# CederGroupHub/sparse-lm

Measured on NVIDIA B200. Metric: cv_grid_fits_per_sec, higher is better.
Workload: dtype f64

## Files before the change

### sparselm_b200/csrc/engine.cu

```cuda
#include <cuda_runtime.h>
#include <float.h>
#include <math.h>
#include <stdint.h>
#include <stdio.h>
#include <stdlib.h>
#include <string.h>

#include <algorithm>
#include <string>
#include <vector>

#include "../../include/sparselm_b200.h"
#include "gemm_f64.cuh"
#include "gemm_f64_tma.cuh"
#include "solver_kernels.cuh"
#include "whiten_kernels.cuh"
#include "cg_kernels.cuh"
#include "coop_kernels.cuh"
#include "newton_kernels.cuh"
#include "select_kernels.cuh"

using namespace slm;

enum { FAM_GRAM = 0, FAM_APPLY = 1, FAM_PROX = 2, FAM_GAP = 3, FAM_SCORE = 4, FAM_LIPS = 5, FAM_COUNT = 6 };
// ... 1776 lines not shown
            LAUNCH_OK("zflags_kernel");
        }
        const bool probe = can_adapt && !check && !coop && !clus && (it == 1 || it == 3 || it == 6);
        const int cw_now = (wide && !check && !probe) ? cw_wide : cw;
        const double* ap_in = fused ? Bc[par] : Z;
        double* ap_out = fused ? GBc[par] : GZ;
        int rc = sparse ? apply_rowsparse(ctx, sp, Kcur, ap_in, ap_out, cw_now, (int)((ldz + cw_now - 1) / cw_now), sidx,
                                          scount, s, algo)
                        : apply_batched(ctx, bt->G_dev, bt->g_stride, bt->pa, p, F, Kcur, ap_in, ldz, ap_out, s, algo);
        if (rc) return rc;
        if ((check || probe) && (can_adapt || (clus_thr > 0 && sparse && F * ncc <= kMaxScount)))
            CUDA_OK(cudaMemcpyAsync(ctx->h_scount, scount, sizeof(int) * (size_t)F * ncc, cudaMemcpyDeviceToHost, s));
        if (probe) {
            CUDA_OK(cudaStreamSynchronize(s));
            decide_width();
        }
        if (check) {
            CUDA_OK(cudaMemsetAsync(ctx->d_counter, 0, sizeof(int) * SLM_MAX_FOLDS, s));
            CUDA_OK(cudaMemsetAsync(ctx->d_ratio, 0, sizeof(unsigned long long), s));
            {
                FamTimer tm(ctx, FAM_GAP, s, 0.0);
                SolveDev spg = sp;
                if (fused) {
                    spg.B = Bc[par];
                    spg.GZ = GBc[par];
                    spg.direct = 1;
                }
                if (grouped)
                    gap_partial_kernel<true><<<cgrid, ST, 0, s>>>(spg, par, 0);
                else
                    gap_partial_kernel<false><<<cgrid, ST, 0, s>>>(spg, par, 0);
                gap_final_kernel<<<fgrid, 128, 0, s>>>(spg, it, 0);
                if (fused) settle_done_kernel<<<mgrid, ST, 0, s>>>(sp, Bc[par], Bc[par ^ 1]);
            }
            LAUNCH_OK("gap kernels");
            ctx->launches++;
            CUDA_OK(cudaMemcpyAsync(ctx->h_counter, ctx->d_counter, sizeof(int) * SLM_MAX_FOLDS,
                                    cudaMemcpyDeviceToHost, s));
            CUDA_OK(cudaMemcpyAsync(ctx->h_ratio, ctx->d_ratio, sizeof(unsigned long long),
                                    cudaMemcpyDeviceToHost, s));
            CUDA_OK(cudaStreamSynchronize(s));
            n_active = 0;
            bool shrink = false;
            for (int f = 0; f < F; ++f) {
                n_active_f[f] = ctx->h_counter[f];
                n_active += n_active_f[f];
                if (round_up(n_active_f[f], 8) < round_up(Kcur[f], 8)) shrink = true;
            }
            next_regular = it + ((n_active * 8 <= Ktot && Ktot >= 16) ? std::max(2, check_every / 2) : check_every);
            if (ctx->trace)
                fprintf(stderr, "[slm] it=%d active=%lld Kmax=%d%s\n", it, n_active, Kmax,
                        coop ? " coop" : (small ? " small" : (clus ? " cluster" : "")));
            if (n_active == 0) break;
            if (clus_thr > 0) {
                bool pays = false;
                if (n_active <= clus_thr && sparse && F * ncc <= kMaxScount) {
                    double bytes = 0.0, flops = 0.0;
                    for (int f = 0; f < F; ++f) {
                        const int Kp = (int)std::min<int64_t>(round_up(n_active_f[f], 8), ldz);
                        for (int cc = 0; cc * cw < Kp; ++cc) {
                            const double sc = (double)std::min<long long>(ctx->h_scount[f * ncc + cc], p);
                            const double ncol = (double)std::min(cw, Kp - cc * cw);
                            bytes += ncol * (double)p * sc * 8.0;
                            flops += 2.0 * ncol * (double)p * sc;
                        }
                    }
                    const int conc = std::max(1, std::min(ctx->sm_count / clus_cs_min, 8 * (16 / clus_cs_min)));
                    const double rounds = (double)((n_active + conc - 1) / conc);
                    const double t_cl = std::max(rounds * 12e-6, bytes / 3.0e12);
                    const double t_ge = 90e-6 + flops / 20e12;
                    pays = t_cl < 0.5 * t_ge;
                }
                if (pays && !clus) {
                    clus = true;
                    interval = check_every;
                    prev_ratio = 0.0;
                } else if (!pays && clus) {
                    clus = false;
                }
            }
            do_compact = shrink && !small && !coop;
            if (small || coop || clus) {
                int step_to = interval;
                double ratio;
                memcpy(&ratio, ctx->h_ratio, sizeof(double));
                if (prev_ratio > 0.0 && ratio > 1.0 && ratio < prev_ratio && it > prev_check) {
                    const double rate = log(prev_ratio / ratio) / (double)(it - prev_check);
                    const double need = 1.15 * log(ratio) / rate + 1.0;
                    if (need < (double)step_to) step_to = std::max(std::max(2, check_every / 2), (int)ceil(need));
                }
                prev_ratio = ratio;
                prev_check = it;
                next_check = it + step_to;
                interval = std::min(interval * 2, 2048);
            }
            if (can_adapt) decide_width();
        }
        {
            FamTimer tm(ctx, FAM_PROX, s, 0.0);
            if (fused) {
                FusedArgs fa;
                fa.Bcur = Bc[par];
                fa.Bnew = Bc[par ^ 1];
                fa.GBcur = GBc[par];
                fa.GBold = GBc[par ^ 1];
                fa.stash = Z;
                fa.it = it;
                fa.use_rst = use_rst;
                use_rst = 0;
                const int rows_lane = bt->max_group > 0 ? (bt->max_group + SUB - 1) / SUB : 8;
                if (!grouped)
                    prox_fused_kernel<false, 1><<<cgrid, ST, 0, s>>>(sp, fa, par);
                else if (rows_lane <= 2)
                    prox_fused_kernel<true, 2><<<cgrid, ST, 0, s>>>(sp, fa, par);
                else if (rows_lane <= 3)
                    prox_fused_kernel<true, 3><<<cgrid, ST, 0, s>>>(sp, fa, par);
                else if (rows_lane <= 5)
                    prox_fused_kernel<true, 5><<<cgrid, ST, 0, s>>>(sp, fa, par);
                else
                    prox_fused_kernel<true, 8><<<cgrid, ST, 0, s>>>(sp, fa, par);
            } else if (ctx->prox2) {
                SolveDev s2 = sp;
                s2.gpt = std::max(1, (Gn + PX_W * kMaxChunks - 1) / (PX_W * kMaxChunks));
                s2.n_chunks = (Gn + PX_W * s2.gpt - 1) / (PX_W * s2.gpt);
                const dim3 cgrid2((unsigned)((Kmax + PX_C - 1) / PX_C), (unsigned)s2.n_chunks, (unsigned)F);
                const dim3 mgrid2((unsigned)((Kmax + PX_C - 1) / PX_C), (unsigned)((p + MOM_ROWS - 1) / MOM_ROWS),
                                  (unsigned)F);
                if (grouped)
                    prox_main2_kernel<true><<<cgrid2, PX_W * PX_C, 0, s>>>(s2, par);
                else
                    prox_main2_kernel<false><<<cgrid2, PX_W * PX_C, 0, s>>>(s2, par);
                prox_momentum2_kernel<<<mgrid2, PX_W * PX_C, 0, s>>>(s2, par);
            } else {
                if (grouped)
                    prox_main_kernel<true><<<cgrid, ST, 0, s>>>(sp, par);
                else
                    prox_main_kernel<false><<<cgrid, ST, 0, s>>>(sp, par);
                prox_momentum_kernel<<<mgrid, ST, 0, s>>>(sp, par);
            }
        }
        LAUNCH_OK("prox kernels");
        ctx->launches++;
        if (do_compact) {
            SolveDev spc = sp;
            if (fused) {
                spc.Z = Bc[par ^ 1];
                spc.B = Bc[par];
                spc.GB = GBc[par];
                restart_reduce_kernel<<<fgrid, 128, 0, s>>>(sp, par);
                use_rst = 1;
            }
            compact_plan_kernel<<<F, 32, 0, s>>>(sp, src, newK);
            scatter_done_kernel<<<mgrid, ST, 0, s>>>(spc, 0);
            compact_move_kernel<<<dim3((unsigned)((p + 127) / 128), 3, (unsigned)F), 128, 0, s>>>(spc, src, newK);
            compact_cols_kernel<<<F, 32, 0, s>>>(sp, src, newK, colmap);
            LAUNCH_OK("compaction kernels");
            ctx->launches += 3;
            Kmax = 0;
            for (int f = 0; f < F; ++f) {
                sp.K[f] = Kcur[f] = n_active_f[f];
                Kmax = std::max(Kmax, Kcur[f]);
            }
            grids(Kmax, cgrid, mgrid, fgrid);
            do_compact = false;
            if (sparse) {
                zflags_kernel<<<zgrid, 256, 0, s>>>(sp, fused ? Bc[par ^ 1] : Z);
                LAUNCH_OK("zflags_kernel");
            }
        }
        if (fused && clus) {
            const int pn = par ^ 1;
            fused_to_classic_kernel<<<mgrid, ST, 0, s>>>(sp, Bc[pn], Bc[par], GBc[par], it + 1, pn, use_rst);
            LAUNCH_OK("fused_to_classic_kernel");
            use_rst = 0;
            fused = false;
            if (sparse) {
                zflags_kernel<<<zgrid, 256, 0, s>>>(sp, Z);
                LAUNCH_OK("zflags_kernel");
            }
        }
    }
    bt->iters_run = it;
    {
        SolveDev spe = sp;
        if (fused) spe.B = Bc[it & 1];
        scatter_done_kernel<<<mgrid, ST, 0, s>>>(spe, 1);
    }
    LAUNCH_OK("scatter_done_kernel");

    SolveDev fin = sp;
    fin.B = bt->B_dev;
    fin.colmap = nullptr;
    for (int f = 0; f < F; ++f) fin.K[f] = bt->K[f];
    grids(Kmax0, cgrid, mgrid, fgrid);
    CUDA_OK(cudaMemcpyAsync(Z, bt->B_dev, state * sizeof(double), cudaMemcpyDeviceToDevice, s));
    if (sparse) {
        zflags_kernel<<<zgrid, 256, 0, s>>>(fin, Z);
        LAUNCH_OK("zflags_kernel");
        int rc = apply_rowsparse(ctx, fin, bt->K, Z, GZ, cw, ncc, sidx, scount, s, 0.0);
        if (rc) return rc;
        CUDA_OK(cudaMemcpyAsync(ctx->h_stat, ctx->d_stat, sizeof(unsigned long long), cudaMemcpyDeviceToHost, s));
    } else {
        int rc = apply_batched(ctx, bt->G_dev, bt->g_stride, bt->pa, p, F, bt->K, Z, ldz, GZ, s, 0.0);
        if (rc) return rc;
    }
    CUDA_OK(cudaMemsetAsync(ctx->d_counter, 0, sizeof(int) * SLM_MAX_FOLDS, s));
    {
        FamTimer tm(ctx, FAM_GAP, s, 0.0);
        if (grouped)
            gap_partial_kernel<true><<<cgrid, ST, 0, s>>>(fin, 0, 1);
        else
            gap_partial_kernel<false><<<cgrid, ST, 0, s>>>(fin, 0, 1);
        gap_final_kernel<<<fgrid, 128, 0, s>>>(fin, it, 1);
    }
    LAUNCH_OK("gap kernels(final)");
    ctx->launches++;
    CUDA_OK(cudaMemcpyAsync(ctx->h_counter, ctx->d_counter, sizeof(int) * SLM_MAX_FOLDS, cudaMemcpyDeviceToHost, s));
    CUDA_OK(cudaStreamSynchronize(s));
    bt->n_unconverged = 0;
    for (int f = 0; f < F; ++f) bt->n_unconverged += ctx->h_counter[f];
    if (sparse) ctx->apply_exec_flops += 2.0 * (double)p * (double)(*ctx->h_stat);
    return 0;
}


static inline int64_t nw_ldh(int64_t p) { return round_up(p, 8); }
static inline int nw_panels(int64_t p) { return (int)((p + NW_NB - 1) / NW_NB); }

size_t slm_newton_workspace(int64_t p, int32_t n_groups, int32_t k, int n_folds) {
    const size_t ldh = (size_t)nw_ldh(p), kk = (size_t)k;
    const size_t ldz = (size_t)round_up(k, 8);
    size_t d = kk * ldh * ldh;
    d += kk * (size_t)nw_panels(p) * NW_NB * NW_NB;
    d += 6 * kk * ldh;
    d += (size_t)round_up((int64_t)(kk * (size_t)n_groups), 2);
    d += 2 * (size_t)n_folds * (size_t)p * ldz;
    return d * sizeof(double) + (4 * kk + kk * ldh + 64) * sizeof(int) + 256;
}

static int newton_step_impl(slm_ctx* ctx, const double* G, int64_t g_stride, int64_t pa, int64_t p, int n_folds,
                            int32_t k, const int32_t* fold_host, const double* nobs_dev, double* X, const double* W2,
                            const double* D2, const double* W1, const int32_t* gptr, const int32_t* gid,
                            int32_t n_groups, void* work, size_t work_bytes, double* out, void* stream) {
    if (!ctx || !G || !fold_host || !nobs_dev || !X || !W2 || !gptr || !gid || !work || !out)
        return fail(ctx, 1, "slm_newton_step: null argument");
    if (k <= 0) return 0;
    if (n_folds < 1 || n_folds > SLM_MAX_FOLDS) return fail(ctx, 1, "slm_newton_step: n_folds out of range");
    if (work_bytes < slm_newton_workspace(p, n_groups, k, n_folds))
        return fail(ctx, 1, "slm_newton_step: workspace too small");
    if (n_groups > 6000) return fail(ctx, 1, "slm_newton_step: too many groups for the line-search kernel");
    cudaStream_t s = (cudaStream_t)stream;
    const int64_t ldv = nw_ldh(p), ldz = round_up(k, 8);
    double* H = (double*)work;
    double* INV = H + (size_t)k * ldv * ldv;
    double* U = INV + (size_t)k * nw_panels(p) * NW_NB * NW_NB;
    double* KK = U + (size_t)k * ldv;
    double* DP = KK + (size_t)k * ldv;
    double* GS = DP + (size_t)k * ldv;
    double* GRAD = GS + (size_t)k * ldv;
    double* DIR = GRAD + (size_t)k * ldv;
    double* NRM = DIR + (size_t)k * ldv;
    double* Z = NRM + (size_t)round_up((int64_t)k * n_groups, 2);
    double* GZ = Z + (size_t)n_folds * p * ldz;
    int* fold_dev = (int*)(GZ + (size_t)n_folds * p * ldz);
    int* slot_dev = fold_dev + k;
    int* info = slot_dev + k;
    int* MS = info + k;
    int* ACT = MS + k;

    std::vector<int32_t> fs(2 * (size_t)k), Kf(n_folds, 0);
    for (int c = 0; c < k; ++c) {
        const int f = fold_host[c];
        if (f < 0 || f >= n_folds) return fail(ctx, 1, "slm_newton_step: fold index out of range");
        fs[c] = f;
        fs[k + c] = Kf[f]++;
    }
    CUDA_OK(cudaMemcpyAsync(fold_dev, fs.data(), sizeof(int32_t) * 2 * (size_t)k, cudaMemcpyHostToDevice, s));
    CUDA_OK(cudaMemsetAsync(info, 0, sizeof(int) * (size_t)k, s));
    CUDA_OK(cudaMemsetAsync(Z, 0, sizeof(double) * (size_t)n_folds * p * ldz, s));

    if (!ctx->newton_smem_set) {
        CUDA_OK(cudaFuncSetAttribute(chol_diag_kernel, cudaFuncAttributeMaxDynamicSharedMemorySize, (int)NW_TILE_SMEM));
        CUDA_OK(cudaFuncSetAttribute(chol_panel_kernel, cudaFuncAttributeMaxDynamicSharedMemorySize, (int)NW_TILE_SMEM));
        CUDA_OK(cudaFuncSetAttribute(newton_linesearch_kernel, cudaFuncAttributeMaxDynamicSharedMemorySize, 98304));
        CUDA_OK(cudaFuncSetAttribute(chol_solve_kernel, cudaFuncAttributeMaxDynamicSharedMemorySize, 98304));
        ctx->newton_smem_set = true;
    }
    const dim3 vgrid((unsigned)((p + NW_T - 1) / NW_T), (unsigned)k);
    newton_prepare_kernel<<<k, NW_T, 0, s>>>((int)p, n_groups, gptr, X, ldv, W2, D2, W1, NRM, U, KK, DP, ACT, MS);
    std::vector<int> ms((size_t)k);
    CUDA_OK(cudaMemcpyAsync(ms.data(), MS, sizeof(int) * (size_t)k, cudaMemcpyDeviceToHost, s));
    newton_pack_kernel<<<vgrid, NW_T, 0, s>>>((int)p, fold_dev, slot_dev, X, ldv, Z, ldz);
    LAUNCH_OK("newton prepare/pack kernels");
    if (int rc = apply_batched(ctx, G, g_stride, pa, p, n_folds, Kf.data(), Z, ldz, GZ, s, -1.0, FAM_LIPS)) return rc;
    newton_grad_kernel<<<vgrid, NW_T, 0, s>>>((int)p, G, g_stride, pa, fold_dev, slot_dev, nobs_dev, X, GZ, ldz, ldv, KK,
                                              DP, W1, GS, GRAD);
    CUDA_OK(cudaStreamSynchronize(s));
    int m_max = 0;
    for (int c = 0; c < k; ++c) m_max = std::max(m_max, ms[c]);
    const int64_t ldh = std::max<int64_t>(8, nw_ldh(m_max));
    const int npan = std::max(1, nw_panels(m_max));
    if (m_max > 0) {
        const dim3 hgrid((unsigned)((ldh + NW_T - 1) / NW_T), (unsigned)ldh, (unsigned)k);
        newton_hessian_kernel<<<hgrid, NW_T, 0, s>>>((int)p, G, g_stride, pa, fold_dev, nobs_dev, gid, U, KK, DP, ldv, ACT, MS,
                                                     H, ldh);
    }
    LAUNCH_OK("newton grad/hessian kernels");
// ... 378 lines not shown
```

### sparselm_b200/csrc/solver_kernels.cuh

```cuda
#pragma once
#include <cuda_runtime.h>
#include <math.h>

#include "../../include/sparselm_b200.h"

namespace slm {

#ifndef SLM_PROX_UR
#define SLM_PROX_UR 1
#endif
#ifndef SLM_PROX_MINB
#define SLM_PROX_MINB 4
#endif
constexpr int SC = 8;
constexpr int SG = 32;
constexpr int ST = SC * SG;
constexpr int kMaxChunks = 64;
constexpr int NQ = 7;
constexpr int MOM_ROWS = 256;

struct SolveDev {
    int F, p, Gn;
    int gpt;
    int n_chunks;
// ... 553 lines not shown
                const int j = j0 + r;
                if (j < jb) {
                    const long long e = sbase + (long long)j * ldz;
                    const double gb = (gz[r] + theta * gbo[r]) * inv1pt;
                    const double v = z[r] - son * (gz[r] - cj[r]);
                    const double u = softt(v, step * w1[r]);
                    if (active) {
                        sp.GB[e] = gb;
                        sp.T[e] = u;
                    }
                    ss += u * u;
                }
            }
        }
        const double nrm = sqrt(ss);
        const double w2 = sp.W2 ? sp.W2[gbase + (long long)g * ldz] : 0.0;
        const double d2 = sp.D2 ? sp.D2[gbase + (long long)g * ldz] : 0.0;
        double scale = nrm > 0.0 ? fmax(0.0, 1.0 - step * w2 / nrm) : 0.0;
        scale = scale / (1.0 + step * d2);
        if (active) {
            for (int j0 = ja; j0 < jb; j0 += PX_UR) {
                double t[PX_UR], z[PX_UR], bo[PX_UR];
#pragma unroll
                for (int r = 0; r < PX_UR; ++r) {
                    const int j = j0 + r;
                    if (j < jb) {
                        const long long e = sbase + (long long)j * ldz;
                        t[r] = sp.T[e];
                        z[r] = sp.Z[e];
                        bo[r] = sp.B[e];
                    }
                }
#pragma unroll
                for (int r = 0; r < PX_UR; ++r) {
                    const int j = j0 + r;
                    if (j < jb) {
                        const double bn = scale * t[r];
                        sp.T[sbase + (long long)j * ldz] = bn;
                        dot += (z[r] - bn) * (bn - bo[r]);
                    }
                }
            }
        }
    }
    red[w][lane] = active ? dot : 0.0;
    __syncthreads();
    if (w == 0 && active) {
        double d = 0.0;
#pragma unroll
        for (int q = 0; q < PX_W; ++q) d += red[q][lane];
        sp.part[(((long long)f * sp.n_chunks + chunk) * NQ + 0) * ldz + k] = d;
    }
}

__global__ void __launch_bounds__(PX_W * PX_C) prox_momentum2_kernel(const __grid_constant__ SolveDev sp, int par) {
    const int f = blockIdx.z;
    const int Kf = sp.K[f];
    const int k0 = blockIdx.x * PX_C;
    if (k0 >= Kf) return;
    const int lane = threadIdx.x & 31, w = threadIdx.x >> 5;
    const int k = k0 + lane;
    const long long ldz = sp.ldz;
    const long long colbase = (long long)f * ldz + k;
    const bool active = (k < Kf) && sp.flag[colbase] == 0;
    const int j0 = blockIdx.y * MOM_ROWS;
    const int j1 = min(j0 + MOM_ROWS, sp.p);
    const int cb0 = blockIdx.x * (PX_C / SC);
    if (__syncthreads_and(!active)) {
        if (sp.zflag)
            for (int e = threadIdx.x; e < (j1 - j0) * (PX_C / SC); e += PX_W * PX_C) {
                const int j = j0 + e / (PX_C / SC), cb = cb0 + e % (PX_C / SC);
                if (cb < sp.nblk) sp.zflag[((long long)f * sp.p + j) * sp.nblk + cb] = 0;
            }
        return;
    }
    double dsum = 0.0;
    if (active)
        for (int ch = 0; ch < sp.n_chunks; ++ch) dsum += sp.part[(((long long)f * sp.n_chunks + ch) * NQ + 0) * ldz + k];
    const double tm = active ? sp.tmom[par][colbase] : 1.0;
    double tn = 0.5 * (1.0 + sqrt(1.0 + 4.0 * tm * tm));
    double th = (tm - 1.0) / tn;
    if (dsum > 0.0) {
        th = 0.0;
        tn = 1.0;
    }
    const long long sbase = (long long)f * sp.p * ldz + k;
#pragma unroll 1
    for (int jj = w; jj < MOM_ROWS; jj += 4 * PX_W) {
        double bn[4], b[4];
        bool inb[4];
#pragma unroll
        for (int r = 0; r < 4; ++r) {
            const int j = j0 + jj + r * PX_W;
            inb[r] = j < j1;
            if (inb[r] && active) {
                const long long e = sbase + (long long)j * ldz;
                bn[r] = sp.T[e];
                b[r] = sp.B[e];
            }
        }
#pragma unroll
        for (int r = 0; r < 4; ++r) {
            const int j = j0 + jj + r * PX_W;
            bool nz = false;
            if (inb[r] && active) {
                const long long e = sbase + (long long)j * ldz;
                const double z = bn[r] + th * (bn[r] - b[r]);
                sp.Z[e] = z;
                sp.B[e] = bn[r];
                nz = z != 0.0;
            }
            if (sp.zflag) {
                const unsigned bal = __ballot_sync(0xffffffffu, nz);
                if ((lane & 7) == 0 && inb[r]) {
                    const int cb = cb0 + (lane >> 3);
                    if (cb < sp.nblk)
                        sp.zflag[((long long)f * sp.p + j) * sp.nblk + cb] = (unsigned char)(((bal >> lane) & 0xffu) != 0u);
                }
            }
        }
    }
    if (active && blockIdx.y == 0 && w == 0) {
        sp.theta[par ^ 1][colbase] = th;
        sp.tmom[par ^ 1][colbase] = tn;
    }
}

__global__ void __launch_bounds__(256) zflags_kernel(const __grid_constant__ SolveDev sp,
                                                     const double* __restrict__ Zsrc) {
    const int f = blockIdx.y;
    const long long i = (long long)blockIdx.x * blockDim.x + threadIdx.x;
    if (i >= (long long)sp.p * sp.nblk) return;
    const int j = (int)(i / sp.nblk), cb = (int)(i - (long long)j * sp.nblk);
    const int Kf = sp.K[f];
    bool nz = false;
    const double* row = Zsrc + ((long long)f * sp.p + j) * sp.ldz;
    for (int k = cb * SC; k < min(cb * SC + SC, Kf); ++k) nz |= row[k] != 0.0;
    sp.zflag[((long long)f * sp.p + j) * sp.nblk + cb] = nz ? 1 : 0;
}

__global__ void __launch_bounds__(1024) support_list_kernel(const __grid_constant__ SolveDev sp, int wb, int ncc,
                                                            int* __restrict__ sidx, int* __restrict__ scount,
                                                            unsigned long long* __restrict__ stat) {
    const int f = blockIdx.y, cc = blockIdx.x;
    const int Kf = sp.K[f];
    const int nb_f = (Kf + SC - 1) / SC;
    const int b0 = cc * wb, b1 = min(b0 + wb, nb_f);
    const int tid = threadIdx.x, lane = tid & 31, warp = tid >> 5;
    int* out = sidx + ((long long)f * ncc + cc) * sp.p;
    if (b0 >= nb_f) {
        if (tid == 0) scount[f * ncc + cc] = 0;
        return;
    }
    __shared__ int wtot[32];
    __shared__ int woff[32];
    __shared__ int base_s, btot;
    if (tid == 0) base_s = 0;
    __syncthreads();
    for (int j0 = 0; j0 < sp.p; j0 += 1024) {
        const int j = j0 + tid;
        bool nz = false;
        if (j < sp.p) {
            const unsigned char* fl = sp.zflag + ((long long)f * sp.p + j) * sp.nblk;
            for (int b = b0; b < b1; ++b) nz |= fl[b] != 0;
        }
        const unsigned bal = __ballot_sync(0xffffffffu, nz);
        if (lane == 0) wtot[warp] = __popc(bal);
        __syncthreads();
        if (warp == 0) {
            int v = wtot[lane], x = v;
#pragma unroll
            for (int o = 1; o < 32; o <<= 1) {
                int y = __shfl_up_sync(0xffffffffu, x, o);
                if (lane >= o) x += y;
            }
            woff[lane] = x - v;
            if (lane == 31) btot = x;
        }
        __syncthreads();
        const int base = base_s;
        if (nz) out[base + woff[warp] + __popc(bal & ((1u << lane) - 1u))] = j;
        __syncthreads();
        if (tid == 0) base_s = base + btot;
        __syncthreads();
    }
    if (tid == 0) {
        scount[f * ncc + cc] = base_s;
        if (stat) atomicAdd(stat, (unsigned long long)base_s * (unsigned long long)(min(b1 * SC, Kf) - b0 * SC));
    }
}

template <bool GROUPED, typename GF, typename WF>
__device__ __forceinline__ double group_dual_newton(unsigned qmask, int ja, int jb, int sub, int rstep, double w2,
                                                    double lo, double hi, GF gfun, WF wfun) {
    double nu = lo;
    for (int it = 0; it < 50; ++it) {
        double s2 = 0.0, sw = 0.0;
        for (int j = ja + sub; j < jb; j += rstep) {
            const double w = wfun(j);
            const double u = gfun(j) - nu * w;
            if (u > 0.0) {
                s2 += u * u;
                sw += w * u;
            }
        }
        if (GROUPED) {
            s2 = sub_sum(qmask, s2);
            sw = sub_sum(qmask, sw);
        }
        const double s = sqrt(s2);
        const double psi = s - nu * w2;
        if (!(psi > 0.0)) break;
        const double dpsi = -sw / s - w2;
        const double nn = nu - psi / dpsi;
        if (!(nn > nu)) break;
        nu = nn;
    }
    double bump = 4e-16;
    for (int t = 0; t < 12; ++t) {
        const double cand = nu * (1.0 + bump);
        double s2 = 0.0;
        for (int j = ja + sub; j < jb; j += rstep) {
            const double u = gfun(j) - cand * wfun(j);
            if (u > 0.0) s2 += u * u;
        }
        if (GROUPED) s2 = sub_sum(qmask, s2);
        if (sqrt(s2) <= cand * w2) return fmin(cand, hi);
        bump *= 8.0;
    }
    return hi;
}

template <bool GROUPED>
__global__ void __launch_bounds__(ST) gap_partial_kernel(const __grid_constant__ SolveDev sp, int par,
                                                         int final_mode) {
    const int f = blockIdx.z, chunk = blockIdx.y;
    const int Kf = sp.K[f];
    const int k0 = blockIdx.x * SC;
    if (k0 >= Kf) return;
    const int c = threadIdx.x % SC, gl = threadIdx.x / SC;
    const int k = k0 + c;
    __shared__ double red[SG][SC];
    const long long ldz = sp.ldz;
    const long long colbase = (long long)f * ldz + k;
    bool active = k < Kf;
    if (active) active = final_mode ? !(sp.skip && sp.skip[colbase]) : (sp.flag[colbase] == 0);
    if (__syncthreads_and(!active)) return;

    const double theta = (active && !final_mode) ? sp.theta[par][colbase] : 0.0;
    const double inv1pt = 1.0 / (1.0 + theta);
    const double* __restrict__ cvec = sp.G + (long long)f * sp.g_stride + (long long)sp.p * sp.pa;
    const double n = sp.n_obs[f];
    const double inv_n = 1.0 / n;
    const int ko = (active && sp.colmap) ? sp.colmap[colbase] : k;
    const int kk = active ? k : 0;
    const long long sbase = (long long)f * sp.p * ldz + kk;
    const long long wbase = (long long)f * sp.p * ldz + (active ? ko : 0);
    const long long gbase = (long long)f * sp.Gn * ldz + (active ? ko : 0);
    const double lam1 = (active && sp.lam1) ? sp.lam1[(long long)f * ldz + ko] : 0.0;
    const int sub = GROUPED ? (gl % SUB) : 0;
    const int gsl = GROUPED ? (gl / SUB) : gl;
    const int gstep = GROUPED ? GPB : SG;
    const int rstep = GROUPED ? SUB : 1;
    const unsigned qmask = 0x01010101u << c;

    auto gb_at = [&](long long e) {
        const double gz = sp.GZ[e];
        return (final_mode || sp.direct) ? gz : (gz + theta * sp.GB[e]) * inv1pt;
    };

    double cb = 0.0, bgb = 0.0, pen = 0.0, ridge = 0.0, lbmax = 0.0;
    for (int i = 0; i < sp.gpt; ++i) {
        const int g = (chunk * sp.gpt + i) * gstep + gsl;
        if (g >= sp.Gn) break;
        const int ja = sp.gptr ? sp.gptr[g] : g;
        const int jb = sp.gptr ? sp.gptr[g + 1] : g + 1;
        const double w2 = sp.W2 ? sp.W2[gbase + (long long)g * ldz] : 0.0;
        const double d2 = sp.D2 ? sp.D2[gbase + (long long)g * ldz] : 0.0;
        double ss = 0.0, gg2 = 0.0, ratio = 0.0, ww2 = 0.0;
        bool anyinf = false;
        for (int j = ja + sub; j < jb; j += rstep) {
            const long long e = sbase + (long long)j * ldz;
            const double gb = gb_at(e);
            const double b = sp.B[e];
            const double cj = cvec[j];
            const double w1 = sp.W1 ? sp.W1[wbase + (long long)j * ldz] : lam1;
            cb += cj * b;
            bgb += b * gb;
            pen += w1 * fabs(b);
            ss += b * b;
            const double gj = fabs((cj - gb) * inv_n - d2 * b);
            gg2 += gj * gj;
            ww2 += w1 * w1;
            if (gj > 0.0) {
                if (w1 > 0.0)
                    ratio = fmax(ratio, gj / w1);
                else
                    anyinf = true;
            }
        }
        if (GROUPED) {
            ss = sub_sum(qmask, ss);
            gg2 = sub_sum(qmask, gg2);
            ww2 = sub_sum(qmask, ww2);
            ratio = sub_max(qmask, ratio);
            anyinf = sub_any(qmask, anyinf);
        }
        if (sub == 0) {
            pen += w2 * sqrt(ss);
            ridge += d2 * ss;
        }
        double lb;
        const double gn = sqrt(gg2);
        if (gg2 == 0.0)
            lb = 0.0;
        else if (w2 <= 0.0)
            lb = anyinf ? INFINITY : ratio;
        else if (ww2 == 0.0)
            lb = gn / w2;
        else
            lb = gn / (w2 + sqrt(ww2));
        lbmax = fmax(lbmax, lb);
    }
    if (!active) lbmax = 0.0;
    const double thr = lanes_max(lbmax, red, gl, c);
    double omega = lbmax;
    for (int i = 0; i < sp.gpt; ++i) {
        const int g = (chunk * sp.gpt + i) * gstep + gsl;
        if (g >= sp.Gn) break;
        const double w2 = sp.W2 ? sp.W2[gbase + (long long)g * ldz] : 0.0;
        const int ja = sp.gptr ? sp.gptr[g] : g;
        const int jb = sp.gptr ? sp.gptr[g + 1] : g + 1;
        const double d2 = sp.D2 ? sp.D2[gbase + (long long)g * ldz] : 0.0;
        auto gfun = [&](int j) {
            const long long e = sbase + (long long)j * ldz;
            return fabs((cvec[j] - gb_at(e)) * inv_n - d2 * sp.B[e]);
        };
        auto wfun = [&](int j) { return sp.W1 ? sp.W1[wbase + (long long)j * ldz] : lam1; };
        double gg2 = 0.0, ratio = 0.0, ww2 = 0.0;
        bool anyinf = false;
        for (int j = ja + sub; j < jb; j += rstep) {
            const double gj = gfun(j), w1 = wfun(j);
            gg2 += gj * gj;
            ww2 += w1 * w1;
            if (gj > 0.0) {
                if (w1 > 0.0)
                    ratio = fmax(ratio, gj / w1);
                else
                    anyinf = true;
            }
        }
        if (GROUPED) {
            gg2 = sub_sum(qmask, gg2);
            ww2 = sub_sum(qmask, ww2);
            ratio = sub_max(qmask, ratio);
            anyinf = sub_any(qmask, anyinf);
        }
        const double gn = sqrt(gg2);
        double hi = w2 > 0.0 ? gn / w2 : 0.0;
        if (!anyinf && ratio < hi) hi = ratio;
        const bool refine = active && w2 > 0.0 && gg2 > 0.0 && ww2 > 0.0 && hi > thr;
        if (refine) {
            const double lo = gn / (w2 + sqrt(ww2));
            omega = fmax(omega, group_dual_newton<GROUPED>(qmask, ja, jb, sub, rstep, w2, lo, hi, gfun, wfun));
        }
    }
    cb = lanes_sum(active ? cb : 0.0, red, gl, c);
    bgb = lanes_sum(active ? bgb : 0.0, red, gl, c);
    pen = lanes_sum(active ? pen : 0.0, red, gl, c);
    ridge = lanes_sum(active ? ridge : 0.0, red, gl, c);
    omega = lanes_max(active ? omega : 0.0, red, gl, c);
    if (active && gl == 0) {
        double* dst = sp.part + (((long long)f * sp.n_chunks + chunk) * NQ) * ldz + k;
        dst[0 * ldz] = cb;
        dst[1 * ldz] = bgb;
        dst[2 * ldz] = pen;
        dst[3 * ldz] = ridge;
        dst[4 * ldz] = omega;
    }
}

__global__ void gap_final_kernel(const __grid_constant__ SolveDev sp, int it, int final_mode) {
    const int f = blockIdx.y;
    const int k = blockIdx.x * blockDim.x + threadIdx.x;
    if (k >= sp.K[f]) return;
    const long long ldz = sp.ldz;
    const long long colbase = (long long)f * ldz + k;
    const bool active = final_mode ? !(sp.skip && sp.skip[colbase]) : (sp.flag[colbase] == 0);
    if (!active) return;
    const int ko = sp.colmap ? sp.colmap[colbase] : k;
    const long long obase = (long long)f * ldz + ko;
    double cb = 0.0, bgb = 0.0, pen = 0.0, ridge = 0.0, omega = 0.0;
    for (int ch = 0; ch < sp.n_chunks; ++ch) {
        const double* src = sp.part + (((long long)f * sp.n_chunks + ch) * NQ) * ldz + k;
        cb += src[0 * ldz];
        bgb += src[1 * ldz];
        pen += src[2 * ldz];
        ridge += src[3 * ldz];
        omega = fmax(omega, src[4 * ldz]);
    }
    const double* Gf = sp.G + (long long)f * sp.g_stride;
    const double n = sp.n_obs[f];
    const double yty = Gf[(long long)sp.p * sp.pa + sp.p];
    const double rr = yty - 2.0 * cb + bgb;
    const double rr_aug = rr + n * ridge;
    const double yr = yty - cb;
    const double P = rr_aug / (2.0 * n) + pen;
    double s = omega > 1.0 ? 1.0 / omega : 1.0;
    if (!(omega < INFINITY)) s = 0.0;
    const double D = (2.0 * s * yr - s * s * rr_aug) / (2.0 * n);
    const double gap = P - D;
    const double scale = fmax(fabs(P), fmax(sp.floor_rel, 4e-15 / sp.tol) * yty / (2.0 * n));
    const bool finite = isfinite(P) && isfinite(gap);
    const bool conv = finite && gap <= sp.tol * scale;
    if (sp.gap) sp.gap[obase] = gap;
    if (sp.primal) sp.primal[obase] = P;
    if (!final_mode) {
        if (conv || !finite) {
            sp.flag[colbase] = 1;
            if (sp.n_iter) sp.n_iter[obase] = it;
            if (sp.status) sp.status[obase] = finite ? 0 : 2;
        } else {
            atomicAdd(sp.counter + f, 1);
            if (sp.ratio) atomicMax(sp.ratio, (unsigned long long)__double_as_longlong(gap / (sp.tol * scale)));
        }
    } else {
        const bool undecided = sp.status ? sp.status[obase] == -1 : true;
        if (undecided && sp.n_iter) sp.n_iter[obase] = it;
        const bool ok = undecided ? conv : (finite && gap <= 4.0 * sp.tol * scale);
        if (sp.status && (undecided || !ok)) sp.status[obase] = !finite ? 2 : (ok ? 0 : 1);
        if (!ok) atomicAdd(sp.counter + f, 1);
    }
}

__global__ void compact_plan_kernel(const __grid_constant__ SolveDev sp, int* __restrict__ src,
                                    int* __restrict__ newK) {
    const int f = blockIdx.x;
    if (threadIdx.x != 0) return;
    const long long base = (long long)f * sp.ldz;
    int kc = 0;
    for (int k = 0; k < sp.K[f]; ++k)
        if (sp.flag[base + k] == 0) src[base + kc++] = k;
    newK[f] = kc;
}

__global__ void __launch_bounds__(ST) scatter_done_kernel(const __grid_constant__ SolveDev sp, int all) {
    const int f = blockIdx.z;
    const int Kf = sp.K[f];
    const int k0 = blockIdx.x * SC;
    if (k0 >= Kf) return;
    const int c = threadIdx.x % SC, r = threadIdx.x / SC;
    const int k = k0 + c;
    if (k >= Kf) return;
    const long long ldz = sp.ldz;
    const long long colbase = (long long)f * ldz + k;
    const int flag = sp.flag[colbase];
    if (flag == 3 || (!all && flag == 0)) return;
    const int ko = sp.colmap ? sp.colmap[colbase] : k;
    const long long sb = (long long)f * sp.p * ldz + k, ob = (long long)f * sp.p * ldz + ko;
    const int j0 = blockIdx.y * MOM_ROWS;
    const int j1 = min(j0 + MOM_ROWS, sp.p);
    for (int j = j0 + r; j < j1; j += SG) sp.Bout[ob + (long long)j * ldz] = sp.B[sb + (long long)j * ldz];
}

__global__ void compact_move_kernel(const __grid_constant__ SolveDev sp, const int* __restrict__ src,
                                    const int* __restrict__ newK) {
    const int f = blockIdx.z, a = blockIdx.y;
    const int j = blockIdx.x * blockDim.x + threadIdx.x;
    if (j >= sp.p) return;
    const int nk = newK[f];
    if (nk == sp.K[f]) return;
    double* arr = a == 0 ? sp.Z : (a == 1 ? sp.B : sp.GB);
    double* row = arr + ((long long)f * sp.p + j) * sp.ldz;
    const int* sf = src + (long long)f * sp.ldz;
    for (int kc = 0; kc < nk; ++kc) row[kc] = row[sf[kc]];
}

__global__ void compact_cols_kernel(const __grid_constant__ SolveDev sp, const int* __restrict__ src,
                                    const int* __restrict__ newK, int* __restrict__ colmap) {
    const int f = blockIdx.x;
    if (threadIdx.x != 0) return;
    const int nk = newK[f];
    if (nk == sp.K[f]) return;
    const long long base = (long long)f * sp.ldz;
    for (int kc = 0; kc < nk; ++kc) {
        const int k = src[base + kc];
        for (int par = 0; par < 2; ++par) {
            sp.theta[par][base + kc] = sp.theta[par][base + k];
            sp.tmom[par][base + kc] = sp.tmom[par][base + k];
        }
        if (sp.rst) sp.rst[base + kc] = sp.rst[base + k];
        colmap[base + kc] = colmap[base + k];
        sp.flag[base + kc] = 0;
    }
}

constexpr int kSmallPMax = 160;

__host__ __device__ inline size_t fista_small_smem(int p, int p32, int nsplit) {
    return sizeof(double) * ((size_t)p * p32 + (size_t)p32 * (2 + nsplit) + 64);
}

template <bool GROUPED>
__global__ void __launch_bounds__(256) fista_small_kernel(const __grid_constant__ SolveDev sp, int par, int n_inner,
                                                          int p32, int nsplit) {
    extern __shared__ __align__(16) double sm[];
    const int f = blockIdx.y, k = blockIdx.x;
    if (k >= sp.K[f]) return;
    const long long ldz = sp.ldz;
    const long long colbase = (long long)f * ldz + k;
    if (sp.flag[colbase] != 0) return;
    const int p = sp.p;
    double* Gs = sm;
    double* zs = Gs + (size_t)p * p32;
    double* us = zs + p32;
    double* parts = us + p32;
    double* red = parts + (size_t)nsplit * p32;
    const int tid = threadIdx.x, nt = blockDim.x;
    const int row = tid % p32, split = tid / p32;
    const bool valid = row < p && split < nsplit;
    const bool owner = valid && split == 0;
    const double* __restrict__ Gf = sp.G + (long long)f * sp.g_stride;
    for (int e = tid; e < p * p; e += nt) {
        const int j = e / p, i = e - j * p;
        Gs[(size_t)j * p32 + i] = Gf[(long long)j * sp.pa + i];
    }
    const int ko = sp.colmap ? sp.colmap[colbase] : k;
    const double n = sp.n_obs[f], step = sp.lips_dev ? 1.0 / sp.lips_dev[f] : sp.step[f];
    const double son = step / n;
    const long long sbase = (long long)f * p * ldz + k;
    double zi = 0.0, bi = 0.0, gbi = 0.0, cj = 0.0, tw1 = 0.0, tw2 = 0.0, rd = 1.0;
    int ja = row, jb = row + 1;
    if (owner) {
        const long long e = sbase + (long long)row * ldz;
        zi = sp.Z[e];
        bi = sp.B[e];
        gbi = sp.GB[e];
        cj = Gf[(long long)p * sp.pa + row];
        const double w1 = sp.W1 ? sp.W1[(long long)f * p * ldz + (long long)row * ldz + ko]
                                : (sp.lam1 ? sp.lam1[(long long)f * ldz + ko] : 0.0);
        tw1 = step * w1;
        int g = row;
        if (GROUPED) {
            int lo = 0, hi = sp.Gn - 1;
            while (lo < hi) {
                const int mid = (lo + hi + 1) >> 1;
                if (sp.gptr[mid] <= row)
                    lo = mid;
                else
                    hi = mid - 1;
            }
            g = lo;
            ja = sp.gptr[g];
            jb = sp.gptr[g + 1];
        }
        const long long gbase = (long long)f * sp.Gn * ldz + (long long)g * ldz + ko;
        tw2 = step * (sp.W2 ? sp.W2[gbase] : 0.0);
        rd = 1.0 / (1.0 + step * (sp.D2 ? sp.D2[gbase] : 0.0));
    }
    if (tid < p32) zs[tid] = owner ? zi : 0.0;
    if (tid == 0) {
        red[32] = sp.theta[par][colbase];
        red[33] = sp.tmom[par][colbase];
    }
    __syncthreads();
    double theta = red[32], tm = red[33];
    const int warp = tid >> 5, lane = tid & 31, nwarp = (nt + 31) >> 5;

#pragma unroll 1
    for (int it = 0; it < n_inner; ++it) {
        double a0 = 0.0, a1 = 0.0;
        if (valid) {
            int j = split;
            for (; j + nsplit < p; j += 2 * nsplit) {
                a0 += Gs[(size_t)j * p32 + row] * zs[j];
                a1 += Gs[(size_t)(j + nsplit) * p32 + row] * zs[j + nsplit];
            }
            if (j < p) a0 += Gs[(size_t)j * p32 + row] * zs[j];
        }
        double gz = a0 + a1;
        if (nsplit > 1) {
            if (valid) parts[(size_t)split * p32 + row] = gz;
            __syncthreads();
            if (owner) {
                gz = parts[row];
                for (int s2 = 1; s2 < nsplit; ++s2) gz += parts[(size_t)s2 * p32 + row];
            }
        }
        double u = 0.0;
        if (owner) {
            gbi = (gz + theta * gbi) / (1.0 + theta);
            u = softt(zi - son * (gz - cj), tw1);
            us[row] = u;
        }
        __syncthreads();
        double bn = 0.0, d = 0.0;
        if (owner) {
            double ss = 0.0;
            if (GROUPED) {
                for (int j = ja; j < jb; ++j) ss += us[j] * us[j];
            } else {
                ss = u * u;
            }
            const double nrm = sqrt(ss);
            const double scale = (nrm > 0.0 ? fmax(0.0, 1.0 - tw2 / nrm) : 0.0) * rd;
            bn = scale * u;
            d = (zi - bn) * (bn - bi);
        }
#pragma unroll
        for (int o = 16; o > 0; o >>= 1) d += __shfl_xor_sync(0xffffffffu, d, o);
        if (lane == 0) red[warp] = d;
        __syncthreads();
        if (tid == 0) {
            double dsum = 0.0;
            for (int w = 0; w < nwarp; ++w) dsum += red[w];
            double tn = 0.5 * (1.0 + sqrt(1.0 + 4.0 * tm * tm));
            double th = (tm - 1.0) / tn;
            if (dsum > 0.0) {
                th = 0.0;
                tn = 1.0;
            }
            red[32] = th;
            red[33] = tn;
        }
        __syncthreads();
        theta = red[32];
        tm = red[33];
        if (owner) {
            zi = bn + theta * (bn - bi);
            bi = bn;
            zs[row] = zi;
        }
        __syncthreads();
    }
    if (owner) {
        const long long e = sbase + (long long)row * ldz;
        sp.Z[e] = zi;
        sp.B[e] = bi;
        sp.GB[e] = gbi;
    }
    if (tid == 0) {
        const int po = par ^ (n_inner & 1);
        sp.theta[po][colbase] = theta;
        sp.tmom[po][colbase] = tm;
    }
}
// ... 3 lines not shown
```

Measured before the change: 18160.

## Warp-parallelize compaction kernels and single-pass support list scan

Result: faster. 18390, median of 6 (+1.3%).

```diff
diff --git a/sparselm_b200/csrc/engine.cu b/sparselm_b200/csrc/engine.cu
--- a/sparselm_b200/csrc/engine.cu
+++ b/sparselm_b200/csrc/engine.cu
@@ -1952,7 +1952,8 @@
             }
             compact_plan_kernel<<<F, 32, 0, s>>>(sp, src, newK);
             scatter_done_kernel<<<mgrid, ST, 0, s>>>(spc, 0);
-            compact_move_kernel<<<dim3((unsigned)((p + 127) / 128), 3, (unsigned)F), 128, 0, s>>>(spc, src, newK);
+            compact_move_kernel<<<dim3((unsigned)((p + MOVE_ROWS - 1) / MOVE_ROWS), 3, (unsigned)F), MOVE_ROWS * 32, 0, s>>>(
+                spc, src, newK);
             compact_cols_kernel<<<F, 32, 0, s>>>(sp, src, newK, colmap);
             LAUNCH_OK("compaction kernels");
             ctx->launches += 3;
diff --git a/sparselm_b200/csrc/solver_kernels.cuh b/sparselm_b200/csrc/solver_kernels.cuh
--- a/sparselm_b200/csrc/solver_kernels.cuh
+++ b/sparselm_b200/csrc/solver_kernels.cuh
@@ -729,41 +729,44 @@
         if (tid == 0) scount[f * ncc + cc] = 0;
         return;
     }
-    __shared__ int wtot[32];
     __shared__ int woff[32];
-    __shared__ int base_s, btot;
-    if (tid == 0) base_s = 0;
+    __shared__ int btot;
+    const int R = (sp.p + 1023) / 1024;
+    const int ja = min(tid * R, sp.p), jb = min(ja + R, sp.p);
+    const unsigned char* fl = sp.zflag + (long long)f * sp.p * sp.nblk;
+    auto on = [&](int j) {
+        bool nz = false;
+        for (int b = b0; b < b1; ++b) nz |= fl[(long long)j * sp.nblk + b] != 0;
+        return nz;
+    };
+    int cnt = 0;
+    for (int j = ja; j < jb; ++j) cnt += on(j) ? 1 : 0;
+    int x = cnt;
+#pragma unroll
+    for (int o = 1; o < 32; o <<= 1) {
+        const int y = __shfl_up_sync(0xffffffffu, x, o);
+        if (lane >= o) x += y;
+    }
+    if (lane == 31) woff[warp] = x;
     __syncthreads();
-    for (int j0 = 0; j0 < sp.p; j0 += 1024) {
-        const int j = j0 + tid;
-        bool nz = false;
-        if (j < sp.p) {
-            const unsigned char* fl = sp.zflag + ((long long)f * sp.p + j) * sp.nblk;
-            for (int b = b0; b < b1; ++b) nz |= fl[b] != 0;
-        }
-        const unsigned bal = __ballot_sync(0xffffffffu, nz);
-        if (lane == 0) wtot[warp] = __popc(bal);
-        __syncthreads();
-        if (warp == 0) {
-            int v = wtot[lane], x = v;
-#pragma unroll
-            for (int o = 1; o < 32; o <<= 1) {
-                int y = __shfl_up_sync(0xffffffffu, x, o);
-                if (lane >= o) x += y;
-            }
-            woff[lane] = x - v;
-            if (lane == 31) btot = x;
-        }
-        __syncthreads();
-        const int base = base_s;
-        if (nz) out[base + woff[warp] + __popc(bal & ((1u << lane) - 1u))] = j;
-        __syncthreads();
-        if (tid == 0) base_s = base + btot;
-        __syncthreads();
-    }
+    if (warp == 0) {
+        const int v = woff[lane];
+        int w = v;
+#pragma unroll
+        for (int o = 1; o < 32; o <<= 1) {
+            const int y = __shfl_up_sync(0xffffffffu, w, o);
+            if (lane >= o) w += y;
+        }
+        woff[lane] = w - v;
+        if (lane == 31) btot = w;
+    }
+    __syncthreads();
+    int pos = woff[warp] + x - cnt;
+    for (int j = ja; j < jb; ++j)
+        if (on(j)) out[pos++] = j;
     if (tid == 0) {
-        scount[f * ncc + cc] = base_s;
-        if (stat) atomicAdd(stat, (unsigned long long)base_s * (unsigned long long)(min(b1 * SC, Kf) - b0 * SC));
+        scount[f * ncc + cc] = btot;
+        if (stat) atomicAdd(stat, (unsigned long long)btot * (unsigned long long)(min(b1 * SC, Kf) - b0 * SC));
     }
 }
 
@@ -1013,12 +1016,19 @@
 __global__ void compact_plan_kernel(const __grid_constant__ SolveDev sp, int* __restrict__ src,
                                     int* __restrict__ newK) {
     const int f = blockIdx.x;
-    if (threadIdx.x != 0) return;
+    const int lane = threadIdx.x;
+    if (lane >= 32) return;
     const long long base = (long long)f * sp.ldz;
+    const int Kf = sp.K[f];
     int kc = 0;
-    for (int k = 0; k < sp.K[f]; ++k)
-        if (sp.flag[base + k] == 0) src[base + kc++] = k;
-    newK[f] = kc;
+    for (int k0 = 0; k0 < Kf; k0 += 32) {
+        const int k = k0 + lane;
+        const bool keep = k < Kf && sp.flag[base + k] == 0;
+        const unsigned bal = __ballot_sync(0xffffffffu, keep);
+        if (keep) src[base + kc + __popc(bal & ((1u << lane) - 1u))] = k;
+        kc += __popc(bal);
+    }
+    if (lane == 0) newK[f] = kc;
 }
 
 __global__ void __launch_bounds__(ST) scatter_done_kernel(const __grid_constant__ SolveDev sp, int all) {
@@ -1040,35 +1050,63 @@
     for (int j = j0 + r; j < j1; j += SG) sp.Bout[ob + (long long)j * ldz] = sp.B[sb + (long long)j * ldz];
 }
 
-__global__ void compact_move_kernel(const __grid_constant__ SolveDev sp, const int* __restrict__ src,
-                                    const int* __restrict__ newK) {
+constexpr int MOVE_ROWS = 8;
+__global__ void __launch_bounds__(MOVE_ROWS * 32) compact_move_kernel(const __grid_constant__ SolveDev sp,
+                                                                      const int* __restrict__ src,
+                                                                      const int* __restrict__ newK) {
     const int f = blockIdx.z, a = blockIdx.y;
-    const int j = blockIdx.x * blockDim.x + threadIdx.x;
+    const int lane = threadIdx.x & 31;
+    const int j = blockIdx.x * MOVE_ROWS + (threadIdx.x >> 5);
     if (j >= sp.p) return;
     const int nk = newK[f];
     if (nk == sp.K[f]) return;
     double* arr = a == 0 ? sp.Z : (a == 1 ? sp.B : sp.GB);
     double* row = arr + ((long long)f * sp.p + j) * sp.ldz;
     const int* sf = src + (long long)f * sp.ldz;
-    for (int kc = 0; kc < nk; ++kc) row[kc] = row[sf[kc]];
+    for (int kc0 = 0; kc0 < nk; kc0 += 32) {
+        const int kc = kc0 + lane;
+        double v = 0.0;
+        if (kc < nk) v = row[sf[kc]];
+        __syncwarp();
+        if (kc < nk) row[kc] = v;
+        __syncwarp();
+    }
 }
 
 __global__ void compact_cols_kernel(const __grid_constant__ SolveDev sp, const int* __restrict__ src,
                                     const int* __restrict__ newK, int* __restrict__ colmap) {
     const int f = blockIdx.x;
-    if (threadIdx.x != 0) return;
+    const int lane = threadIdx.x;
+    if (lane >= 32) return;
     const int nk = newK[f];
     if (nk == sp.K[f]) return;
     const long long base = (long long)f * sp.ldz;
-    for (int kc = 0; kc < nk; ++kc) {
-        const int k = src[base + kc];
-        for (int par = 0; par < 2; ++par) {
-            sp.theta[par][base + kc] = sp.theta[par][base + k];
-            sp.tmom[par][base + kc] = sp.tmom[par][base + k];
-        }
-        if (sp.rst) sp.rst[base + kc] = sp.rst[base + k];
-        colmap[base + kc] = colmap[base + k];
-        sp.flag[base + kc] = 0;
+    for (int kc0 = 0; kc0 < nk; kc0 += 32) {
+        const int kc = kc0 + lane;
+        const bool on = kc < nk;
+        double th0 = 0.0, th1 = 0.0, tm0 = 0.0, tm1 = 0.0, rs = 0.0;
+        int cm = 0;
+        if (on) {
+            const long long k = base + src[base + kc];
+            th0 = sp.theta[0][k];
+            th1 = sp.theta[1][k];
+            tm0 = sp.tmom[0][k];
+            tm1 = sp.tmom[1][k];
+            if (sp.rst) rs = sp.rst[k];
+            cm = colmap[k];
+        }
+        __syncwarp();
+        if (on) {
+            const long long e = base + kc;
+            sp.theta[0][e] = th0;
+            sp.theta[1][e] = th1;
+            sp.tmom[0][e] = tm0;
+            sp.tmom[1][e] = tm1;
+            if (sp.rst) sp.rst[e] = rs;
+            colmap[e] = cm;
+            sp.flag[e] = 0;
+        }
+        __syncwarp();
     }
 }
 
```
